# ZcsrenlongZ/Deblur4DGS

Measured on AMD Instinct MI355X. Metric: Gaussians/s fwd+bwd, 288x512, N_exposure=8, higher is better.
Workload: dtype f32; 1 GPU; cfg2: 300000 Gaussians (300000 dynamic), 6 motion bases, 512x288, N_exposure=8, 3+depth channels, fwd+bwd to all leaves; gaussians=300000, exposure_subsamples=8, parallelism=1 GPU, lazy_sort=off (auto), pre_roll_steps=30

## Files before the change

deblur4dgs_amd/csrc/binning.hip:

```cpp
#include "common.h"

namespace {

struct EmitArgs {
  D4gsDims d;
  const float *depths;
  const int32_t *tile_rects;
  const int32_t *tiles_touched;
  const int32_t *isect_offsets;
  int32_t *isect_offsets_out;
  const int32_t *chunk_base;
  int nchunks;
  int32_t *tile_cursor;
  const int32_t *tile_offsets;
  uint64_t *keys;
  int32_t *gid_of_emit;
  int tw, th;
  const int64_t *n_dev;
  int64_t cap, max_hint;
  int use_lds;
  LazyWs lazy;
  const uint64_t *tile_masks;
};

template <int EMIT_PER_THREAD, int LZ>
__global__ void __launch_bounds__(D4GS_CHUNK_THREADS) k_emit(const EmitArgs a) {
  extern __shared__ int bins[];
  if (lists_overflowed(a.n_dev, a.cap, a.max_hint)) return;
  constexpr bool LAZY = LZ != 0;
  const int tiles = a.tw * a.th, tid = threadIdx.x;
  const int s = blockIdx.x % a.d.S, chunk = blockIdx.x / a.d.S;
  const int tbase = s * tiles, n_tiles_all = a.d.S * tiles;
  const bool lds = a.use_lds;
  __shared__ int fbox[4];
  if (lds) {
    for (int z = tid; z < tiles; z += D4GS_CHUNK_THREADS) bins[z] = 0;
    if (LZ == 2 && tid == 0) fbox[0] = fbox[1] = 1 << 30, fbox[2] = fbox[3] = -1;
    __syncthreads();
  }
// ... 98 lines not shown
      __syncthreads();
      int base = 0, tot = 0;
#pragma unroll
      for (int w = 0; w < D4GS_CHUNK_THREADS / 64; w++) {
        const int x = wsum[w];
        base += w < wave ? x : 0;
        tot += x;
      }
      ebase[q] = (uint32_t)(carry + base + inc - cnt[q]);
      carry += tot;
      __syncthreads();
      const int g = (chunk * EMIT_PER_THREAD + q) * D4GS_CHUNK_THREADS + tid;
      if (g < a.d.N) a.isect_offsets_out[(int64_t)s * a.d.N + g] = (int32_t)ebase[q];
    }
  }
#pragma unroll
  for (int q = 0; q < EMIT_PER_THREAD; q++) {
    if (cnt[q] == 0) continue;
    const int g = (chunk * EMIT_PER_THREAD + q) * D4GS_CHUNK_THREADS + tid;
    const int64_t i = (int64_t)s * a.d.N + g;
    const int x0 = rx[q] & 0xffff, x1 = rx[q] >> 16, y0 = ry[q] & 0xffff, y1 = ry[q] >> 16;
    const uint64_t hi = (uint64_t)__float_as_uint(dep[q]) << 32;
    uint32_t e = (LZ != 2 && a.nchunks) ? ebase[q] : (uint32_t)a.isect_offsets[i];
    auto put = [&](int t) {
      if (LAZY && !taken(bkq[q], t)) return;
      const int slot = (LAZY || lds) ? atomicAdd(&bins[t], 1)
                                     : a.tile_offsets[tbase + t] + atomicAdd(a.tile_cursor + n_tiles_all + tbase + t, 1);
      a.keys[slot] = hi | e;
      a.gid_of_emit[e] = g;
    };
    if (msk[q]) {
      for (uint64_t m = msk[q]; m; m &= m - 1, e++) {
        const int b = __ffsll((long long)m) - 1;
        put((y0 + (b >> 3)) * a.tw + x0 + (b & 7));
      }
      continue;
    }
    for (int ty = y0; ty < y1; ty++)
      for (int tx = x0; tx < x1; tx++, e++) put(ty * a.tw + tx);
  }
}

__device__ __forceinline__ void bitonic_step(uint64_t *key, int P, int n, int k, int j) {
  for (int t = threadIdx.x; t < (P >> 1); t += blockDim.x) {
    const int blk = t / j, off = t - blk * j;
    const int i = blk * 2 * j + off;
    const int l = (j == (k >> 1)) ? (blk * 2 * j + (2 * j - 1 - off)) : (i + j);
    if (l < n) {
      const uint64_t x = key[i], y = key[l];
      if (x > y) key[i] = y, key[l] = x;
    }
  }
// ... 88 lines not shown
    reg_plain<NV, 1>(v);
    chunk_plain<32, NV>(v, lane);
  }
  if constexpr (NV >= 8) {
    reg_flip<NV, 8>(v);
    reg_plain<NV, 2>(v);
    chunk_plain<32, NV>(v, lane);
  }
}
constexpr int CNV = 8, CHUNK = 64 * CNV;

struct SortArgs {
  const int32_t *tile_offsets;
  uint64_t *keys;
  const int32_t *gid_of_emit;
  int32_t *sorted_gid;
  int32_t *sorted_emit;
  int lo, cap;
  const int64_t *n_dev;
  int64_t n_cap, max_hint;
  int n_lists;
  const int32_t *lazy_near, *lazy_flag;
  int pass;
};
__device__ __forceinline__ bool lazy_range(const SortArgs &a, int t, int &base, int &n) {
  if (a.pass == 1) n = min(n, a.lazy_near[t]);
  else if (a.pass == 2) {
    const int nn = a.lazy_near[t];
    if (nn >= n || a.lazy_flag[t] != 1) return false;
    base += nn, n -= nn;
  }
  return true;
}

__device__ __forceinline__ void put_sorted(const SortArgs &a, int at, uint64_t key) {
  const uint32_t e = (uint32_t)key;
  a.sorted_emit[at] = (int32_t)e;
  a.sorted_gid[at] = a.gid_of_emit[e];
}

template <int NV>
__device__ __forceinline__ void wave_sort_list(const SortArgs &a, int base, int n, int lane) {
  uint64_t v[NV];
  const uint64_t *gk = a.keys + base;
#pragma unroll
  for (int u = 0; u < NV; u++) v[u] = (u * 64 + lane < n) ? gk[u * 64 + lane] : ~0ull;
  chunk_sort<NV>(v, lane);
#pragma unroll
  for (int u = 0; u < NV; u++)
    if (u * 64 + lane < n) put_sorted(a, base + u * 64 + lane, v[u]);
}
__device__ __forceinline__ void wave_sort_list(const SortArgs &a, int base, int n, int lane) {
  if (n <= 64) wave_sort_list<1>(a, base, n, lane);
  else if (n <= 128) wave_sort_list<2>(a, base, n, lane);
  else if (n <= 256) wave_sort_list<4>(a, base, n, lane);
  else wave_sort_list<8>(a, base, n, lane);
}
template <int NV>
__device__ __forceinline__ void sort_list_lds(const SortArgs &a, uint64_t *key, int base, int n) {
// ... 76 lines not shown
    if (threadIdx.x < 64) wave_sort_list(a, base, n, threadIdx.x);
    return;
  }
  if (a.cap >= 0) {
    sort_list_lds(a, skeys, base, n);
  } else {
    uint64_t *gk = a.keys + base;
    bitonic_sort(gk, n);
    for (int p = threadIdx.x; p < n; p += blockDim.x) put_sorted(a, base + p, gk[p]);
  }
}


int launch_sorts(const D4gsDims *dims, const FrontPlan &fp, const D4gsProjOut *proj, const D4gsIsect *isect, int pass, hipStream_t stream) {
  const int n_tiles = fp.n_tiles;
  LazyWs lw{};
  if (pass) lw = d4gs_lazy_carve(proj->lazy_ws, dims->S, fp.tiles);
  (void)hipFuncSetAttribute((const void *)k_tile_sort, hipFuncAttributeMaxDynamicSharedMemorySize, 16384 * 8);
  const int64_t longest = isect->max_tile_count > 0 ? isect->max_tile_count : isect->n_isect;
  const bool merge_short = pass == 0 && longest > CHUNK && isect->n_isect >= (int64_t)768 * n_tiles;
  static const bool no_long = getenv("D4GS_SORT_NO_MERGE_LONG") != nullptr;
  const bool merge_long = !merge_short && !no_long && longest > CHUNK && pass == 0 && isect->n_isect < (int64_t)640 * n_tiles;
  SortArgs s{proj->tile_offsets, isect->keys, isect->gid_of_emit, isect->sorted_gid, isect->sorted_emit,
             0, CHUNK, proj->n_isect, isect->n_isect, isect->max_tile_count, n_tiles, lw.near, lw.flag, pass};
  if (!merge_short) {
    if (merge_long) D4GS_LAUNCH("k_tile_sort_w", k_tile_sort_w<true>, dim3((n_tiles + 3) / 4), dim3(256), 4 * CHUNK * 8, stream, s);
    else D4GS_LAUNCH("k_tile_sort_w", k_tile_sort_w<false>, dim3((n_tiles + 3) / 4), dim3(256), 0, stream, s);
  }
  const int classes[6][3] = {{merge_short ? 0 : CHUNK, 2048, 256}, {2048, 4096, 512}, {4096, 8192, 1024}, {8192, 16384, 1024}, {16384, -1, 1024}};
  for (int c = merge_long ? 1 : 0; c < 5; c++) {
    if (longest <= classes[c][0]) break;
    s.lo = classes[c][0], s.cap = classes[c][1];
    const size_t lds = classes[c][1] > 0 ? (size_t)classes[c][1] * 8 : 0;
    D4GS_LAUNCH("k_tile_sort", k_tile_sort, dim3(n_tiles), dim3(classes[c][2]), lds, stream, s);
  }
  return d4gs_check_launch("k_tile_sort");
}

EmitArgs emit_args(const D4gsDims *dims, const FrontPlan &fp, const D4gsProjOut *proj, const D4gsIsect *isect) {
  EmitArgs e;
  e.d = *dims;
  e.depths = proj->depths;
  e.tile_rects = proj->tile_rects;
  e.tiles_touched = proj->tiles_touched;
  e.isect_offsets = proj->isect_offsets;
  e.isect_offsets_out = proj->isect_offsets, e.chunk_base = proj->scan_ws, e.nchunks = fp.fused_chunks;
  e.tile_cursor = proj->tile_counts;
  e.tile_masks = (dims->flags & D4GS_EXACT_TILES) ? proj->tile_masks : nullptr;
  e.tile_offsets = proj->tile_offsets;
  e.keys = isect->keys;
  e.gid_of_emit = isect->gid_of_emit;
  e.tw = fp.tw, e.th = fp.th;
  e.n_dev = proj->n_isect, e.cap = isect->n_isect, e.max_hint = isect->max_tile_count;
  e.use_lds = fp.hist_in_lds;
  e.lazy = LazyWs{};
  return e;
}

int launch_emit(const EmitArgs &e, const FrontPlan &fp, int lz, hipStream_t stream) {
  const size_t ebytes = fp.hist_in_lds ? sizeof(int) * (size_t)fp.tiles * (lz ? 2 : 1) : 0;
  d4gs_with_pt(fp.pt, [&](auto pt) {
    constexpr int PT = decltype(pt)::value;
    d4gs_launch_chunks("k_emit", lz == 0 ? k_emit<PT, 0> : lz == 1 ? k_emit<PT, 1> : k_emit<PT, 2>, fp, ebytes, stream, e);
  });
  return d4gs_check_launch("k_emit");
}

}

int d4gs_bin_sort_impl(const D4gsDims *dims, const D4gsProjOut *proj, const D4gsIsect *isect, hipStream_t stream) {
  if (isect->n_isect <= 0) return D4GS_OK;
  if (isect->n_isect >= (int64_t)0x7fffffff) {
    d4gs_set_error("n_isect=%lld exceeds int32 indexing", (long long)isect->n_isect);
    return D4GS_ECAPACITY;
// ... 21 lines not shown
```

deblur4dgs_amd/csrc/capi.hip:

```cpp
#include <stdarg.h>
#include <stdio.h>
#include <string.h>

#include <stdint.h>

#include "common.h"

static thread_local char g_err[512] = "";

#include <mutex>
#include <string>
#include <vector>
namespace {
struct ProfRec {
  const char *name;
  hipEvent_t a, b;
};
int g_prof_on = 0;
std::vector<ProfRec> g_prof;
std::mutex g_prof_mu;
}

ProfScope::ProfScope(const char *name, hipStream_t s) : slot(-1), stream(s) {
  if (!g_prof_on) return;
// ... 46 lines not shown
  const bool flag = (d->flags & D4GS_ANTIALIASED) != 0;
  if (flag && !compensations) {
    d4gs_set_error("%s: D4GS_ANTIALIASED needs D4gsProjOut.compensations", who);
    return D4GS_EINVAL;
  }
  if (!flag && compensations) {
    d4gs_set_error("%s: D4gsProjOut.compensations given without D4GS_ANTIALIASED in dims->flags", who);
    return D4GS_EINVAL;
  }
  return D4GS_OK;
}

static int check_dims(const D4gsDims *d) {
  if (!d) {
    d4gs_set_error("dims is NULL");
    return D4GS_EINVAL;
  }
  if (d->D == 0 && d->depth_mode == D4GS_DEPTH_NONE) {
    d4gs_set_error("bad dims: D == 0 needs depth_mode D4GS_DEPTH_D or D4GS_DEPTH_ED (the depth-only render modes)");
    return D4GS_EINVAL;
  }
  if (d->N < 0 || d->S <= 0 || d->width <= 0 || d->height <= 0 || d->D < 0) {
    d4gs_set_error("bad dims N=%d S=%d W=%d H=%d D=%d", d->N, d->S, d->width, d->height, d->D);
    return D4GS_EINVAL;
  }
  if (d->G < 0 || d->G > d->N || (d->G > 0 && (d->K <= 0 || d->K > D4GS_MAX_K || d->T <= 0))) {
    d4gs_set_error("bad motion dims G=%d K=%d (max %d) T=%d", d->G, d->K, D4GS_MAX_K, d->T);
    return D4GS_EINVAL;
  }
  return D4GS_OK;
}

extern "C" {

int d4gs_version(void) { return D4GS_VERSION; }

__global__ void k_copy_counts(const int64_t *__restrict__ n_isect, int64_t *__restrict__ host_pinned) {
  if (threadIdx.x < 4) __hip_atomic_store(host_pinned + threadIdx.x, n_isect[threadIdx.x], __ATOMIC_RELAXED, __HIP_MEMORY_SCOPE_SYSTEM);
}
}
int d4gs_copy_counts_impl(const int64_t *n_isect, int64_t *host_pinned, hipStream_t stream) {
  if (!n_isect || !host_pinned) {
    d4gs_set_error("d4gs_copy_counts: NULL argument");
    return D4GS_EINVAL;
  }
  hipPointerAttribute_t at{};
// ... 474 lines not shown
```

deblur4dgs_amd/csrc/frame.hip:

```cpp
#include "common.h"

namespace {

struct Carve {
  char *base;
  size_t off;
  template <typename T>
  T *take(size_t n) {
    off = (off + 255) & ~(size_t)255;
    T *p = base ? reinterpret_cast<T *>(base + off) : nullptr;
    off += n * sizeof(T);
    return p;
  }
};

struct FrameBufs {
  D4gsProjOut proj;
  D4gsIsect isect;
  D4gsRaster raster;
  float *v_renders, *v_alphas, *isect_grad, *v_conics, *v_depths, *v_opac_act, *v_ctab, *partials;
  uint8_t *isect_live;
  int8_t *blend_win;
  size_t bytes;
  size_t fwd_bytes;
// ... 43 lines not shown
    d4gs_set_error("%s: S=%d sub-samples with a blended frame, the one-call frame takes at most %d (its winner map holds one signed byte "
                   "per pixel and channel); use the staged entry points", who, d->S, D4GS_FRAME_BLEND_MAX_S);
    return D4GS_EINVAL;
  }
  if (!in || !io || !ws || !io->renders || !io->alphas || !io->means2d || !io->radii || !io->n_isect ||
      (io->blended && !io->acc) || !in->means || !in->quats || !in->scales || !in->opacities || !in->colors || !in->viewmat ||
      !in->Kmat || (d->G > 0 && (!in->motion_coefs || !in->rots || !in->transls || !in->times)) || d->N == 0) {
    d4gs_set_error("%s: NULL required buffer", who);
    return D4GS_EINVAL;
  }
  if (((uintptr_t)ws & 255) != 0) {
    d4gs_set_error("%s: the workspace must be 256-byte aligned", who);
    return D4GS_EINVAL;
  }
  const FrameBufs need = carve(d, cap, nullptr);
  if (ws_bytes < (forward_only ? need.fwd_bytes : need.bytes)) {
    d4gs_set_error("%s: workspace of %zu bytes, need %zu (%s)", who, ws_bytes, forward_only ? need.fwd_bytes : need.bytes,
                   forward_only ? "d4gs_frame_workspace_bytes_fwd; d4gs_backward needs d4gs_frame_workspace_bytes" : "d4gs_frame_workspace_bytes");
    return D4GS_ECAPACITY;
  }
  return D4GS_OK;
}

void bind_io(FrameBufs &b, const D4gsFrameIO *io, int64_t cap, int64_t max_hint) {
  b.proj.means2d = io->means2d, b.proj.radii = io->radii, b.proj.n_isect = io->n_isect;
  b.isect.n_isect = cap > 0 ? cap : 1, b.isect.max_tile_count = max_hint, b.isect.near_target = io->near_target;
  b.raster.background = io->background, b.raster.render_colors = io->renders, b.raster.render_alphas = io->alphas;
}

}

extern "C" {

size_t d4gs_frame_workspace_bytes(const D4gsDims *dims, int64_t isect_capacity) {
  D4gsSizes z;
  if (d4gs_query_sizes(dims, &z)) return 0;
  if (dims->D == 0) {
    frame_refuses_depth_only("d4gs_frame_workspace_bytes");
    return 0;
  }
  return carve(dims, isect_capacity, nullptr).bytes;
}

size_t d4gs_frame_workspace_bytes_fwd(const D4gsDims *dims, int64_t isect_capacity) {
  D4gsSizes z;
  if (d4gs_query_sizes(dims, &z)) return 0;
  if (dims->D == 0) {
    frame_refuses_depth_only("d4gs_frame_workspace_bytes_fwd");
    return 0;
  }
  return carve(dims, isect_capacity, nullptr).fwd_bytes;
}

int d4gs_forward(const D4gsDims *dims, const D4gsProjIn *in, const D4gsFrameIO *io, void *ws, size_t ws_bytes,
                 int64_t isect_capacity, int64_t max_tile_hint, void *stream_) {
  int rc = check_frame("d4gs_forward", dims, in, io, ws, ws_bytes, isect_capacity, true);
  if (rc) return rc;
  hipStream_t stream = (hipStream_t)stream_;
  if (io->counts_pinned) {
    hipPointerAttribute_t at{};
    if (hipPointerGetAttributes(&at, io->counts_pinned) != hipSuccess || at.type != hipMemoryTypeHost) {
      (void)hipGetLastError();
      d4gs_set_error("d4gs_forward: io->counts_pinned is not pinned host memory");
      return D4GS_EINVAL;
    }
  }
  FrameBufs b = carve(dims, isect_capacity, ws);
  bind_io(b, io, isect_capacity, max_tile_hint);
  if ((rc = d4gs_project_fwd_impl(dims, in, &b.proj, stream))) return rc;
  if (isect_capacity < 0)
    return io->counts_pinned ? d4gs_copy_counts_impl(io->n_isect, io->counts_pinned, stream) : D4GS_OK;
  if ((rc = d4gs_bin_sort_impl(dims, &b.proj, &b.isect, stream))) return rc;
  if ((rc = d4gs_raster_fwd_impl(dims, &b.proj, &b.isect, &b.raster, stream))) return rc;
  if (io->blended) {
    rc = d4gs_blend_fwd_impl(dims->S, (int64_t)dims->width * dims->height, d4gs_nch(dims), io->policy, io->renders, io->alphas, io->blended,
                             io->acc, b.blend_win, stream,
                             io->n_isect, io->counts_pinned);
  } else if (io->counts_pinned) {
    rc = d4gs_copy_counts_impl(io->n_isect, io->counts_pinned, stream);
  }
  return rc;
}

int d4gs_backward(const D4gsDims *dims, const D4gsProjIn *in, const D4gsFrameIO *io, const D4gsFrameGrads *g,
                  const D4gsLeafGrads *leaf, void *ws, size_t ws_bytes, int64_t isect_capacity, int64_t max_tile_hint,
                  void *stream_) {
  int rc = check_frame("d4gs_backward", dims, in, io, ws, ws_bytes, isect_capacity);
  if (rc) return rc;
  if (!g || !leaf || !g->v_means2d || !leaf->v_means || !leaf->v_quats || !leaf->v_scales || !leaf->v_opacities ||
      !leaf->v_colors || (dims->G > 0 && (!leaf->v_motion_coefs || !leaf->v_rots || !leaf->v_transls)) ||
      (io->blended ? (!g->v_blended && !g->v_acc && !g->v_renders && !g->v_alphas) : !g->v_renders)) {
    d4gs_set_error("d4gs_backward: NULL gradient buffer (a blended frame takes any of v_blended, v_acc, v_renders, v_alphas; an "
                   "unblended one v_renders [+ v_alphas])");
    return D4GS_EINVAL;
  }
  if ((rc = d4gs_check_absgrad("d4gs_backward", dims, g->v_means2d_abs, g->stats_absgrad))) return rc;
  hipStream_t stream = (hipStream_t)stream_;
  FrameBufs b = carve(dims, isect_capacity, ws);
  bind_io(b, io, isect_capacity, max_tile_hint);
  const float *v_renders = g->v_renders, *v_alphas = g->v_alphas;
  const int nch = d4gs_nch(dims);
  const bool fuse_blend = io->blended && !g->v_renders && !g->v_alphas && dims->D <= 5;
  BlendAdj ba{};
  if (fuse_blend) {
    ba.v_blended = g->v_blended, ba.v_acc = g->v_acc, ba.win = b.blend_win;
    for (int c = 0; c < nch; c++)
      if (io->policy && io->policy[c] != 0) ba.non_mean |= (uint64_t)1 << c;
    v_renders = nullptr, v_alphas = nullptr;
  } else if (io->blended) {
    if ((rc = d4gs_blend_bwd_add_impl(dims->S, (int64_t)dims->width * dims->height, nch, io->policy, io->renders, io->blended,
                                      g->v_blended, g->v_acc, b.v_renders, b.v_alphas, g->v_renders, g->v_alphas, stream,
                                      b.blend_win)))
      return rc;
    v_renders = b.v_renders, v_alphas = b.v_alphas;
  }
  D4gsRasterGrads rg{};
  rg.v_render_colors = v_renders, rg.v_render_alphas = v_alphas, rg.isect_grad = b.isect_grad, rg.isect_live = b.isect_live;
  rg.v_means2d = g->v_means2d, rg.v_conics = b.v_conics, rg.v_depths = b.v_depths, rg.v_opac_act = b.v_opac_act;
  rg.v_ctab = b.v_ctab;
  rg.stats_grad_norm_acc = g->stats_grad_norm_acc, rg.stats_vis_count = g->stats_vis_count;
  rg.stats_max_radii = g->stats_max_radii, rg.stats_batch_size = g->stats_batch_size;
  rg.stats_update_max_radii = g->stats_update_max_radii, rg.row_mode = g->row_mode;
// ... 13 lines not shown
```

deblur4dgs_amd/csrc/host.h:

```cpp
#pragma once
#include <hip/hip_runtime_api.h>
#include <stddef.h>
#include <stdint.h>

#include "../../include/d4gs.h"

void d4gs_set_error(const char *fmt, ...);
int d4gs_check_launch(const char *what);
int d4gs_check_absgrad(const char *who, const D4gsDims *d, const float *v_means2d_abs, int32_t stats_absgrad);
int d4gs_check_antialiased(const char *who, const D4gsDims *d, const float *compensations);
int d4gs_copy_counts_impl(const int64_t *n_isect, int64_t *host_pinned, hipStream_t stream);

int d4gs_project_fwd_impl(const D4gsDims *dims, const D4gsProjIn *in, const D4gsProjOut *out, hipStream_t stream);
int d4gs_project_bwd_impl(const D4gsDims *dims, const D4gsProjIn *in, const D4gsProjOut *proj, const float *v_means2d,
                          const float *v_conics, const float *v_depths, const float *v_opac_act, const float *v_ctab,
                          const D4gsLeafGrads *grads, hipStream_t stream);
int d4gs_poses_fwd_impl(const D4gsDims *dims, const D4gsProjIn *in, const D4gsPoses *out, hipStream_t stream);
int d4gs_poses_bwd_impl(const D4gsDims *dims, const D4gsProjIn *in, const D4gsPoses *v_out, const D4gsLeafGrads *grads,
                        hipStream_t stream);
size_t d4gs_poses_bwd_partials_bound(const D4gsDims *d);
int d4gs_bases_table_launch(const D4gsDims *dims, const D4gsProjIn *in, float *btab, hipStream_t stream);
inline int d4gs_tiles_across(int pixels) { return (pixels + D4GS_TILE - 1) / D4GS_TILE; }
inline int d4gs_nch(const D4gsDims *d) { return d->D + (d->depth_mode != D4GS_DEPTH_NONE ? 1 : 0); }

constexpr int D4GS_CHUNK_THREADS = 1024;
static_assert(D4GS_CHUNK_THREADS % 64 == 0 && D4GS_CHUNK_THREADS <= 1024, "whole waves, one workgroup");
struct FrontPlan {
  int tw, th, tiles;
  int n_tiles;
  bool hist_in_lds;
  bool count_apart;
  int pt, per_block, nchunks , blocks ;
  int fused_chunks;
};
FrontPlan d4gs_front_plan(const D4gsDims *d);

int d4gs_bin_sort_impl(const D4gsDims *dims, const D4gsProjOut *proj, const D4gsIsect *isect, hipStream_t stream);
bool d4gs_lazy_on(const D4gsDims *d, const D4gsProjOut *out, const FrontPlan &fp);
int d4gs_lazy_pivot_launch(const D4gsDims *d, const D4gsProjOut *out, const FrontPlan &fp, int64_t near_target, hipStream_t stream);
int d4gs_lazy_far_sort(const D4gsDims *dims, const D4gsProjOut *proj, const D4gsIsect *isect, hipStream_t stream);

struct BlendAdj {
  const float *v_blended;
  const float *v_acc;
  const int8_t *win;
  uint64_t non_mean;
};
int d4gs_raster_fwd_impl(const D4gsDims *dims, const D4gsProjOut *proj, const D4gsIsect *isect, const D4gsRaster *r,
                         hipStream_t stream);
int d4gs_raster_bwd_impl(const D4gsDims *dims, const D4gsProjOut *proj, const D4gsIsect *isect, const D4gsRaster *r,
                         const D4gsRasterGrads *g, const BlendAdj *blend, hipStream_t stream);
int64_t d4gs_seg_state_elems(const D4gsDims *d);
bool d4gs_seg_on(const D4gsDims *d, const D4gsIsect *isect, const D4gsRaster *r);

int d4gs_blend_fwd_impl(int32_t S, int64_t P, int32_t C, const int32_t *policy, const float *renders, const float *alphas,
                        float *out, float *acc, int8_t *win, hipStream_t stream, const int64_t *n_isect = nullptr,
                        int64_t *counts_pinned = nullptr);
// ... 44 lines not shown
```

deblur4dgs_amd/csrc/project_fwd.hip:

```cpp
#include <stdlib.h>

#include "common.h"

namespace {

struct FwdArgs {
  D4gsDims d;
  D4gsProjIn in;
  D4gsProjOut out;
  int tw, th;
  int count_apart;
  int use_table;
};

__device__ __forceinline__ void preblend_bases(const FwdArgs &a, float *Bs) {
#pragma clang fp contract(off)
  const int K = a.d.K, T = a.d.T;
  for (int idx = threadIdx.x; idx < a.d.S * K * 9; idx += blockDim.x) {
    int s = idx / (K * 9), r = idx - s * K * 9, k = r / 9, j = r - k * 9;
    const TimeSlot ts = d4gs_time_slot(a.in.times[s], T);
    const float w = ts.w;
    const int f = ts.f, c = ts.c;
    float vf, vc;
    if (j < 3) {
// ... 655 lines not shown
  static const bool force_in_kernel = getenv("D4GS_COUNT_IN_PROJECT") != nullptr;
  static const bool no_fused_scan = getenv("D4GS_NO_FUSED_SCAN") != nullptr;
  FrontPlan p;
  p.tw = d4gs_tiles_across(d->width), p.th = d4gs_tiles_across(d->height);
  p.tiles = p.tw * p.th, p.n_tiles = d->S * p.tiles;
  p.hist_in_lds = sizeof(int) * (size_t)p.tiles <= 64 * 1024;
  p.count_apart = p.hist_in_lds && d->N > 0 && !force_in_kernel;
  auto blocks_at = [&](int pt) { return (((int64_t)d->N + (int64_t)pt * D4GS_CHUNK_THREADS - 1) / ((int64_t)pt * D4GS_CHUNK_THREADS)) * d->S; };
  p.pt = 4;
  if (blocks_at(4) < 256) {
    p.pt = 1;
  } else if (!(d->flags & D4GS_LAZY_SORT)) {
    for (int pt = 2; pt <= 6; pt++)
      if (blocks_at(pt) <= 512) {
        p.pt = pt;
        break;
      }
  }
  p.per_block = D4GS_CHUNK_THREADS * p.pt;
  p.nchunks = (d->N + p.per_block - 1) / p.per_block;
  p.blocks = p.nchunks * d->S;
  const bool fits = (size_t)p.blocks + 1 <= d4gs_scan_ws_elems((int64_t)d->S * d->N);
  p.fused_chunks = p.count_apart && !no_fused_scan && fits ? p.nchunks : 0;
  return p;
}

bool d4gs_lazy_on(const D4gsDims *d, const D4gsProjOut *out, const FrontPlan &fp) {
  if (!(d->flags & D4GS_LAZY_SORT) || !out->lazy_ws) return false;
  return fp.count_apart && sizeof(int) * (size_t)fp.tiles * (1 + d4gs_lazy_buckets(fp.tiles)) <= 150 * 1024;
}
int d4gs_lazy_pivot_launch(const D4gsDims *d, const D4gsProjOut *out, const FrontPlan &fp, int64_t near_target, hipStream_t stream) {
  const int target = near_target > 0 ? (int)(near_target > (1 << 20) ? (1 << 20) : near_target) : 1024;
  D4GS_LAUNCH("k_lazy_pivot", k_lazy_pivot, dim3((fp.n_tiles + 255) / 256), dim3(256), 0, stream, d4gs_lazy_carve(out->lazy_ws, d->S, fp.tiles),
              fp.n_tiles, target);
  return d4gs_check_launch("k_lazy_pivot");
}

static size_t fwd_lds_bytes(const D4gsDims *dims) {
  if (dims->G <= 0) return 0;
  return sizeof(float) * (((size_t)dims->S * dims->K * 9 + 3) & ~(size_t)3) + sizeof(float) * (size_t)dims->K * D4GS_PROJ_BLOCK;
}

int d4gs_poses_fwd_impl(const D4gsDims *dims, const D4gsProjIn *in, const D4gsPoses *out, hipStream_t stream) {
  PosesArgs a;
  a.d = *dims;
  a.in = *in;
// ... 90 lines not shown
```

deblur4dgs_amd/csrc/raster_bwd.hip:

```cpp
#include <stdlib.h>

#include <type_traits>

#include "composite.h"

namespace {

struct RasterBwdArgs {
  int N, S, width, height, tw, th;
  int ed;
  const float *geom;
  const float *ctab;
  const float *background;
  const int32_t *tile_offsets;
  const int32_t *sorted_gid;
  const int32_t *sorted_emit;
  const float *out;
  const float *alphas;
  const int32_t *last_ids;
  const float *final_T;
  const float *v_out;
  const float *v_alphas;
  float *isect_grad;
  uint8_t *live;
  int sparse;
  const int64_t *n_dev;
  int64_t cap, max_hint;
  const float *seg_state;
  int fuse_blend;
  BlendAdj blend;
#ifdef D4GS_TRACE
  unsigned long long *trace;
#endif
};
#ifdef D4GS_TRACE
#define D4GS_TRACE_BEGIN const unsigned long long _t0 = wall_clock64();
#define D4GS_TRACE_END(n_)                                                                                     \
  if (a.trace && threadIdx.x == 0) {                                                                           \
    unsigned long long *tr = a.trace + (size_t)blockIdx.x * 4;                                                 \
// ... 119 lines not shown
      if (last >= end) {
        const float *sf = a.seg_state + (size_t)t * D4GS_SEG_MAX * (1 + NCH) * 256 + ((y - ty * D4GS_TILE) * D4GS_TILE + (x - tx * D4GS_TILE));
        const float *sb = sf + (size_t)(seg + 1) * (1 + NCH) * 256;
        T = sb[0];
#pragma unroll
        for (int c = 0; c < NCH; c++) bsum = __builtin_fmaf(vo[c], sf[(1 + c) * 256] - sb[(1 + c) * 256], bsum);
        last = end - 1;
      }
    }
  }
  int whi = last < start ? start - 1 : last;
  int wq = whi;
#pragma unroll
  for (int o = 1; o <= 16; o = o == 2 ? 8 : o << 1) wq = max(wq, __shfl_xor(wq, o));
  const int wq0 = __builtin_amdgcn_readlane(wq, 0), wq1 = __builtin_amdgcn_readlane(wq, 4), wq2 = __builtin_amdgcn_readlane(wq, 32),
            wq3 = __builtin_amdgcn_readlane(wq, 36);
#pragma unroll
  for (int o = 32; o > 0; o >>= 1) whi = max(whi, __shfl_xor(whi, o));
  whi = min(whi, end - 1);
  if (lane == 0) shi[wv] = whi;
  __syncthreads();
  const int hi = max(max(shi[0], shi[1]), max(shi[2], shi[3]));
  const size_t inst_base = (size_t)s * a.N;
  float *myslab = sgrad + wv * NB * RP;
  const int wvs = __builtin_amdgcn_readfirstlane(wv);
  float afrag[MC ? 16 : 1];
  float *myfac = sfac + (MC ? wv * 64 * FS : 0);
  int *myhit = shit + (MC ? wv * MH : 0);
  int nh = 0;
  if constexpr (MC > 0) {
    static_assert(256 * MC <= 4 * NB * RP, "exchange buffer");
#pragma unroll
    for (int c = 0; c < MC; c++) sgrad[tid * MC + c] = vo[c];
    __syncthreads();
#pragma unroll
    for (int kk = 0; kk < 16; kk++) afrag[kk] = sgrad[(wv * 64 + 4 * kk + (lane >> 4)) * MC + (lane & 15)];
  }
  auto flush = [&](int nhits) {
    if constexpr (MC > 0) {
      __builtin_amdgcn_wave_barrier();
      f32x4 acc0 = {0.f, 0.f, 0.f, 0.f}, acc1 = {0.f, 0.f, 0.f, 0.f};
      const float *bp = myfac + (lane >> 4) * FS + (lane & (MH - 1));
      float bv[16];
#pragma unroll
      for (int kk = 0; kk < 16; kk++) bv[kk] = bp[4 * kk * FS];
#pragma unroll
      for (int kk = 0; kk < 16; kk += 2) {
        acc0 = __builtin_amdgcn_mfma_f32_16x16x4f32(afrag[kk], bv[kk], acc0, 0, 0, 0);
        acc1 = __builtin_amdgcn_mfma_f32_16x16x4f32(afrag[kk + 1], bv[kk + 1], acc1, 0, 0, 0);
      }
      acc0 += acc1;
      const int n = lane & 15;
      if (n < nhits) {
        float *dst = myslab + myhit[n] * RP + CB + (lane >> 4) * 4;
        dst[0] = acc0[0], dst[1] = acc0[1], dst[2] = acc0[2], dst[3] = acc0[3];
      }
      __builtin_amdgcn_wave_barrier();
    }
  };
  if (!a.sparse)
    for (int idx = hi + 1 + tid; idx < end; idx += 256) {
      float *dst = a.isect_grad + (size_t)a.sorted_emit[idx] * RW;
#pragma unroll
      for (int r = 0; r < RW; r++) dst[r] = 0.f;
    }

  float vab = va - bsum;
  for (int bh = hi; bh >= start; bh -= NB) {
    __syncthreads();
    int emit = -1;
    if (tid < NB) {
      const int idx = bh - tid;
      if (idx >= start) {
        const int gid = a.sorted_gid[idx];
        emit = a.sorted_emit[idx];
        const float4 *gp = reinterpret_cast<const float4 *>(a.geom + (inst_base + gid) * D4GS_GEOM_STRIDE);
        const float4 q0 = gp[0], q1 = gp[1];
        sg0[tid] = q0;
        sg1[tid] = stage_conic(q1.x, q1.y, q1.z, __builtin_amdgcn_rcpf(q0.z));
        const float tau = D4GS_ALPHA_TAU(q0.z);
        D4GS_TIGHT_EXTENTS(ex, ey, tau, q1.x, q1.y, q1.z)
        if constexpr (W4)
          sbox[tid] = ex < 0.f ? d4gs_pack_box(1e30f, -1e30f, 1e30f, -1e30f)
                               : d4gs_pack_box(q0.x - ex - tx0f, q0.x + ex - tx0f, q0.y - ey - ty0f, q0.y + ey - ty0f);
        else
          sbox[tid] = ex < 0.f ? make_float4(1e30f, -1e30f, 1e30f, -1e30f)
                               : make_float4(q0.x - ex, q0.x + ex, q0.y - ey, q0.y + ey);
        const float4 *cp = reinterpret_cast<const float4 *>(a.ctab + (size_t)gid * DP);
#pragma unroll
        for (int v = 0; v < DV; v++) {
          float4 c4 = cp[v];
          if constexpr (DEPTH && (D & 3) != 0) {
            if (v == D / 4) (&c4.x)[D & 3] = q0.w;
          }
          scol[tid * DV + v] = c4;
        }
      }
    }
    for (int z = tid; z < NB * RP; z += 256) reinterpret_cast<float4 *>(sgrad)[z] = make_float4(0.f, 0.f, 0.f, 0.f);
    __syncthreads();
// ... 419 lines not shown
  a.v_opac_act[g] = vo;
#pragma unroll
  for (int c = 0; c < DP; c++) a.v_ctab[(size_t)g * DP + c] = c < D ? vc[c < D ? c : 0] : 0.f;
}

static bool choose_sparse(int row_mode, int64_t n_isect, int64_t n_inst, bool lazy) {
  if (lazy) return true;
  if (row_mode == D4GS_ROWS_DENSE) return false;
  if (row_mode == D4GS_ROWS_SPARSE) return true;
  return n_isect >= 6 * (n_inst > 0 ? n_inst : 1);
}

template <int D, bool DEPTH, bool ABS, bool AA>
int launch_bwd(RasterBwdArgs &a, GatherArgs &ga, const GatherAA &gaa, int64_t n_isect, int row_mode, bool lazy, hipStream_t stream) {
  const int n_tiles = a.S * a.tw * a.th;
  const int blocks = ((n_tiles + 7) / 8) * 8;
  bool launched = false;
  a.sparse = ga.sparse = choose_sparse(row_mode, n_isect, (int64_t)a.S * a.N, lazy) ? 1 : 0;
#ifdef D4GS_VARIANTS
  static const bool wave_per_tile = getenv("D4GS_BWD_WAVE_PER_TILE") != nullptr;
  static const bool use_mfma = getenv("D4GS_BWD_MFMA") != nullptr;
  if constexpr (D > 0) {
    if (!ABS && (wave_per_tile || use_mfma)) {
      constexpr int R = 6 + D + (DEPTH ? 1 : 0);
      a.sparse = ga.sparse = 0;
      if (wave_per_tile) {
        hipError_t e = hipMemsetAsync(a.isect_grad, 0, sizeof(float) * (size_t)R * (size_t)(n_isect > 0 ? n_isect : 1), stream);
        if (e != hipSuccess) {
          d4gs_set_error("hipMemsetAsync(isect_grad): %s", hipGetErrorString(e));
          return D4GS_ELAUNCH;
        }
      }
      if (n_isect > 0) {
        if (wave_per_tile) D4GS_LAUNCH("k_raster_bwd", (k_raster_bwd<D, DEPTH>), dim3(blocks), dim3(64), 0, stream, a);
        else D4GS_LAUNCH("k_raster_bwd_m", (k_raster_bwd_m<D, DEPTH>), dim3(blocks), dim3(256), 0, stream, a);
      }
      launched = true;
    }
  }
#endif
  if (!launched) {
    if (a.sparse) {
      hipError_t e = hipMemsetAsync(a.live, 0, (((size_t)(n_isect > 0 ? n_isect : 1)) + 3) & ~(size_t)3, stream);
      if (e != hipSuccess) {
        d4gs_set_error("hipMemsetAsync(isect_live): %s", hipGetErrorString(e));
        return D4GS_ELAUNCH;
// ... 22 lines not shown
    else D4GS_GATHER(true, 1);
  } else {
    if (slots == 4) D4GS_GATHER(false, 4);
    else if (slots == 2) D4GS_GATHER(false, 2);
    else D4GS_GATHER(false, 1);
  }
#undef D4GS_GATHER
  return d4gs_check_launch("k_gather");
}

}

int d4gs_raster_bwd_impl(const D4gsDims *dims, const D4gsProjOut *proj, const D4gsIsect *isect, const D4gsRaster *r,
                         const D4gsRasterGrads *g, const BlendAdj *blend, hipStream_t stream) {
  RasterBwdArgs a;
  a.fuse_blend = blend != nullptr;
  a.blend = blend ? *blend : BlendAdj{};
  a.N = dims->N, a.S = dims->S, a.width = dims->width, a.height = dims->height;
  const FrontPlan fp = d4gs_front_plan(dims);
  a.tw = fp.tw, a.th = fp.th;
  a.ed = dims->depth_mode == D4GS_DEPTH_ED;
  a.geom = proj->geom, a.ctab = proj->ctab, a.background = r->background;
  a.tile_offsets = proj->tile_offsets, a.sorted_gid = isect->sorted_gid, a.sorted_emit = isect->sorted_emit;
  a.out = r->render_colors, a.alphas = r->render_alphas, a.last_ids = r->last_ids, a.final_T = r->final_T;
  a.v_out = g->v_render_colors, a.v_alphas = g->v_render_alphas, a.isect_grad = g->isect_grad, a.live = g->isect_live;
  a.n_dev = proj->n_isect, a.cap = isect->n_isect, a.max_hint = isect->max_tile_count;
  a.seg_state = d4gs_seg_on(dims, isect, r) ? r->seg_state : nullptr;
#ifdef D4GS_TRACE
  a.trace = getenv("D4GS_TRACE_PTR") ? (unsigned long long *)strtoull(getenv("D4GS_TRACE_PTR"), nullptr, 0) : nullptr;
#endif
  GatherArgs ga;
  ga.n_dev = proj->n_isect, ga.cap = isect->n_isect, ga.max_hint = isect->max_tile_count;
  ga.rows = isect->n_isect > 0 ? isect->n_isect : 1;
  ga.live = g->isect_live;
  ga.N = dims->N, ga.S = dims->S, ga.D = dims->D, ga.DP = (dims->D + 3) & ~3;
  ga.depth = dims->depth_mode != D4GS_DEPTH_NONE;
  ga.tiles_touched = proj->tiles_touched, ga.isect_offsets = proj->isect_offsets, ga.isect_grad = g->isect_grad;
  ga.v_means2d = g->v_means2d, ga.v_conics = g->v_conics, ga.v_depths = g->v_depths, ga.v_opac_act = g->v_opac_act;
  ga.v_ctab = g->v_ctab;
  ga.radii = proj->radii, ga.stats_acc = g->stats_grad_norm_acc, ga.stats_vis = g->stats_vis_count;
  ga.stats_mr = g->stats_max_radii, ga.update_mr = g->stats_update_max_radii;
  ga.sx = (float)dims->width / 2.0f * (float)g->stats_batch_size * (float)dims->S;
  ga.sy = (float)dims->height / 2.0f * (float)g->stats_batch_size * (float)dims->S;
  const bool absg = (dims->flags & D4GS_ABSGRAD) != 0;
  ga.v_means2d_abs = absg ? g->v_means2d_abs : nullptr, ga.stats_abs = absg && g->stats_absgrad;
  ga.max_wh = (float)(dims->width > dims->height ? dims->width : dims->height);
// ... 117 lines not shown
```

deblur4dgs_amd/csrc/raster_fwd.hip:

```cpp
#include <stdlib.h>

#include "composite.h"

namespace {

struct RasterFwdArgs {
  int N, S, width, height, tw, th;
  int ed;
  const float *geom;
  const float *ctab;
  const float *background;
  const int32_t *tile_offsets;
  const int32_t *sorted_gid;
  float *out;
  float *alphas;
  int32_t *last_ids;
  float *final_T;
  int64_t *n_dev;
  int64_t cap, max_hint;
  float *seg_state;
  const int32_t *lazy_near;
  int32_t *lazy_flag;
  int lazy_pass;
  int block_filter;
#ifdef D4GS_TRACE
  unsigned long long *trace;
#endif
};
#ifdef D4GS_TRACE
#define D4GS_TCLK(v_) const unsigned long long v_ = wall_clock64();
#define D4GS_TADD(acc_, a_, b_) acc_ += (b_) - (a_);
// ... 96 lines not shown
  } else if (a.lazy_pass == 2 && !a.lazy_flag[t]) return;
  const size_t inst_base = (size_t)s * a.N;
  const int seglen = SEG ? d4gs_seg_len(end_full - start) : 0;
  float *seg_px = SEG ? a.seg_state + (size_t)t * D4GS_SEG_MAX * (1 + NCH) * 256 + ((y - ty * D4GS_TILE) * D4GS_TILE + (x - tx * D4GS_TILE)) : nullptr;
  auto seg_store = [&](int k) {
    if (inside) {
      float *p = seg_px + (size_t)k * (1 + NCH) * 256;
      p[0] = T;
#pragma unroll
      for (int c = 0; c < NCH; c++) p[(1 + c) * 256] = chan(c);
    }
  };
  for (int b = start; b < end; b += FBE) {
    if (__syncthreads_and(done)) break;
    D4GS_TCLK(_ta)
    const int idx = b + tid - (NULL0 ? 1 : 0);
    if (NULL0 && tid == 0) {
      sg0[0] = make_float4(0.f, 0.f, 0.f, 0.f);
      sg1[0] = make_float4(0.f, 0.f, 0.f, 0.f);
      sbox[0] = BoxT<PB>::pack(1e30f, -1e30f, 1e30f, -1e30f);
#pragma unroll
      for (int v = 0; v < DV; v++) scol[v] = make_float4(0.f, 0.f, 0.f, 0.f);
    } else if (tid < FB && idx < end) {
      const int gid = a.sorted_gid[idx];
      const float4 *gp = reinterpret_cast<const float4 *>(a.geom + (inst_base + gid) * D4GS_GEOM_STRIDE);
      const float4 q0 = gp[0], q1 = gp[1];
      sg0[tid] = q0;
      const float tau = d4gs_alpha_tau(q0.z);
      sg1[tid] = stage_conic(q1.x, q1.y, q1.z, tau * 1.4426950408889634f);
      D4GS_TIGHT_EXTENTS(ex, ey, tau, q1.x, q1.y, q1.z)
      sbox[tid] = ex < 0.f ? BoxT<PB>::pack(1e30f, -1e30f, 1e30f, -1e30f) : BoxT<PB>::pack(q0.x - ex - tx0f, q0.x + ex - tx0f, q0.y - ey - ty0f, q0.y + ey - ty0f);
      const float4 *cp = reinterpret_cast<const float4 *>(a.ctab + (size_t)gid * DP);
#pragma unroll
      for (int v = 0; v < DV; v++) scol[tid * DV + v] = cp[v];
    }
    __syncthreads();
    D4GS_TCLK(_tb)
    D4GS_TADD(_ts, _ta, _tb)
    const bool wave_live = __builtin_amdgcn_ballot_w64(done) != ~0ull;
    const int nb = wave_live ? min(FBE, end - b) + (NULL0 ? 1 : 0) : 0;
    int c0 = 0, c1 = 0, c2 = 0, c3 = 0;
    if constexpr (NARROW) {
      if (lane * 16 < 4 * FB) reinterpret_cast<uint4 *>(wlist)[lane] = make_uint4(0u, 0u, 0u, 0u);
      __builtin_amdgcn_wave_barrier();
    }
#pragma unroll
    for (int k = 0; k < FB / 64; k++) {
// ... 194 lines not shown
  raster_fwd_r_body<D, DEPTH>(a);
}
template <int D, bool DEPTH>
__global__ void __launch_bounds__(256) __attribute__((amdgpu_waves_per_eu(D == 16 ? 6 : 1, D == 16 ? 6 : 10))) k_raster_fwd_r(const RasterFwdArgs a) {
  raster_fwd_r_body<D, DEPTH>(a);
}
template <int D, bool DEPTH>
__global__ void __launch_bounds__(256) __attribute__((amdgpu_waves_per_eu(8, 8))) k_raster_fwd_rs8(const RasterFwdArgs a) {
  raster_fwd_r_body<D, DEPTH, true>(a);
}
template <int D, bool DEPTH>
__global__ void __launch_bounds__(256) __attribute__((amdgpu_waves_per_eu(D == 16 ? 6 : 1, D == 16 ? 6 : 10))) k_raster_fwd_rs(const RasterFwdArgs a) {
  raster_fwd_r_body<D, DEPTH, true>(a);
}

template <int D, bool DEPTH>
int launch_fwd(const RasterFwdArgs &a, hipStream_t stream) {
  const int n_tiles = a.S * a.tw * a.th;
  const int blocks = ((n_tiles + 7) / 8) * 8;
#ifdef D4GS_VARIANTS
  static const bool wave_per_tile = getenv("D4GS_FWD_WAVE_PER_TILE") != nullptr;
  static const bool quads = getenv("D4GS_FWD_QUADS") != nullptr;
  if constexpr (D > 0) {
    if (wave_per_tile) {
      D4GS_LAUNCH("k_raster_fwd", (k_raster_fwd<D, DEPTH>), dim3(blocks), dim3(64), 0, stream, a);
      return d4gs_check_launch("k_raster_fwd");
    }
    if (quads) {
      D4GS_LAUNCH("k_raster_fwd_q", (k_raster_fwd_q<D, DEPTH>), dim3(blocks), dim3(256), 0, stream, a);
      return d4gs_check_launch("k_raster_fwd_q");
    }
  }
#endif
  if (a.seg_state) {
    if constexpr (D <= 4) D4GS_LAUNCH("k_raster_fwd_r", (k_raster_fwd_rs8<D, DEPTH>), dim3(blocks), dim3(256), 0, stream, a);
    else D4GS_LAUNCH("k_raster_fwd_r", (k_raster_fwd_rs<D, DEPTH>), dim3(blocks), dim3(256), 0, stream, a);
    return d4gs_check_launch("k_raster_fwd_r");
  }
  if constexpr (D <= 4) D4GS_LAUNCH("k_raster_fwd_r", (k_raster_fwd_r8<D, DEPTH>), dim3(blocks), dim3(256), 0, stream, a);
  else D4GS_LAUNCH("k_raster_fwd_r", (k_raster_fwd_r<D, DEPTH>), dim3(blocks), dim3(256), 0, stream, a);
  return d4gs_check_launch("k_raster_fwd_r");
}

}

int64_t d4gs_seg_state_elems(const D4gsDims *d) {
// ... 1 lines not shown
  if (n_tiles > (d->D <= 4 ? D4GS_SEG_TILES_MAX_NARROW : D4GS_SEG_TILES_MAX)) return 0;
  return n_tiles * D4GS_SEG_MAX * (1 + d4gs_nch(d)) * 256;
}
bool d4gs_seg_on(const D4gsDims *d, const D4gsIsect *isect, const D4gsRaster *r) {
  const char *env = getenv("D4GS_SEG");
  if (!r->seg_state || d4gs_seg_state_elems(d) == 0 || (env && env[0] == '0')) return false;
#ifdef D4GS_VARIANTS
  if (getenv("D4GS_FWD_WAVE_PER_TILE") || getenv("D4GS_FWD_QUADS") || getenv("D4GS_BWD_WAVE_PER_TILE") || getenv("D4GS_BWD_MFMA"))
    return false;
#endif
  if (env && env[0] == '1') return true;
  return isect->max_tile_count > D4GS_SEG_UNIT;
}

int d4gs_raster_fwd_impl(const D4gsDims *dims, const D4gsProjOut *proj, const D4gsIsect *isect, const D4gsRaster *r,
                         hipStream_t stream) {
  RasterFwdArgs a;
  a.N = dims->N, a.S = dims->S, a.width = dims->width, a.height = dims->height;
  const FrontPlan fp = d4gs_front_plan(dims);
  a.tw = fp.tw, a.th = fp.th;
  a.ed = dims->depth_mode == D4GS_DEPTH_ED;
  a.geom = proj->geom, a.ctab = proj->ctab, a.background = r->background;
  a.tile_offsets = proj->tile_offsets, a.sorted_gid = isect->sorted_gid;
  a.n_dev = proj->n_isect, a.cap = isect->n_isect, a.max_hint = isect->max_tile_count;
  a.out = r->render_colors, a.alphas = r->render_alphas, a.last_ids = r->last_ids, a.final_T = r->final_T;
  a.seg_state = d4gs_seg_on(dims, isect, r) ? r->seg_state : nullptr;
  a.lazy_near = nullptr, a.lazy_flag = nullptr, a.lazy_pass = 0;
  const char *bf = getenv("D4GS_BLOCK_FILTER");
  a.block_filter = !(bf && bf[0] == '0');
  const bool lazy = d4gs_lazy_on(dims, proj, fp) && isect->n_isect > 0;
  if (lazy) {
    const LazyWs lw = d4gs_lazy_carve(proj->lazy_ws, dims->S, fp.tiles);
    a.lazy_near = lw.near, a.lazy_flag = lw.flag, a.lazy_pass = 1;
  }
#ifdef D4GS_TRACE
  a.trace = getenv("D4GS_TRACE_FWD_PTR") ? (unsigned long long *)strtoull(getenv("D4GS_TRACE_FWD_PTR"), nullptr, 0) : nullptr;
#endif
  const bool dep = dims->depth_mode != D4GS_DEPTH_NONE;
  auto launch = [&](const RasterFwdArgs &aa) -> int {
#define D4GS_CASE(DD)                                                   \
  case DD:                                                              \
    return dep ? launch_fwd<DD, true>(aa, stream) : launch_fwd<DD, false>(aa, stream);
    switch (dims->D) {
      case 0:
        if (dep) return launch_fwd<0, true>(aa, stream);
        d4gs_set_error("D = 0 needs a depth mode (the depth-only composite)");
// ... 39 lines not shown
```

Baseline: 253.7 million Gaussians/s.

## Pack gaussian id and per-gaussian ordinal into sort key low word

In the one-call frame path, the low 32 bits of each intersection key hold the gaussian id shifted left plus a per-gaussian tile ordinal, instead of a global emit index. This drops the gid_of_emit scatter in emit, the gather through gid_of_emit in the sort, and the sorted_emit writes. Backward rebuilds the emit index from isect_offsets plus the ordinal when it needs it. It only applies when N and the tile count fit together in 32 bits and lazy sort is off, and the reference raster variants are rejected when it is active.

```diff
diff --git a/deblur4dgs_amd/csrc/binning.hip b/deblur4dgs_amd/csrc/binning.hip
--- a/deblur4dgs_amd/csrc/binning.hip
+++ b/deblur4dgs_amd/csrc/binning.hip
@@ -15,6 +15,7 @@
   const int32_t *tile_offsets;
   uint64_t *keys;
   int32_t *gid_of_emit;
+  int ordbits;
   int tw, th;
   const int64_t *n_dev;
   int64_t cap, max_hint;
@@ -159,12 +160,14 @@
     const int x0 = rx[q] & 0xffff, x1 = rx[q] >> 16, y0 = ry[q] & 0xffff, y1 = ry[q] >> 16;
     const uint64_t hi = (uint64_t)__float_as_uint(dep[q]) << 32;
     uint32_t e = (LZ != 2 && a.nchunks) ? ebase[q] : (uint32_t)a.isect_offsets[i];
+    const bool packed = !LAZY && a.ordbits != 0;
+    if (packed) e = (uint32_t)g << a.ordbits;
     auto put = [&](int t) {
       if (LAZY && !taken(bkq[q], t)) return;
       const int slot = (LAZY || lds) ? atomicAdd(&bins[t], 1)
                                      : a.tile_offsets[tbase + t] + atomicAdd(a.tile_cursor + n_tiles_all + tbase + t, 1);
       a.keys[slot] = hi | e;
-      a.gid_of_emit[e] = g;
+      if (!packed) a.gid_of_emit[e] = g;
     };
     if (msk[q]) {
       for (uint64_t m = msk[q]; m; m &= m - 1, e++) {
@@ -299,6 +302,7 @@
   int n_lists;
   const int32_t *lazy_near, *lazy_flag;
   int pass;
+  int packed;
 };
 __device__ __forceinline__ bool lazy_range(const SortArgs &a, int t, int &base, int &n) {
   if (a.pass == 1) n = min(n, a.lazy_near[t]);
@@ -312,6 +316,10 @@
 
 __device__ __forceinline__ void put_sorted(const SortArgs &a, int at, uint64_t key) {
   const uint32_t e = (uint32_t)key;
+  if (a.packed) {
+    a.sorted_gid[at] = (int32_t)e;
+    return;
+  }
   a.sorted_emit[at] = (int32_t)e;
   a.sorted_gid[at] = a.gid_of_emit[e];
 }
@@ -434,7 +442,7 @@
   static const bool no_long = getenv("D4GS_SORT_NO_MERGE_LONG") != nullptr;
   const bool merge_long = !merge_short && !no_long && longest > CHUNK && pass == 0 && isect->n_isect < (int64_t)640 * n_tiles;
   SortArgs s{proj->tile_offsets, isect->keys, isect->gid_of_emit, isect->sorted_gid, isect->sorted_emit,
-             0, CHUNK, proj->n_isect, isect->n_isect, isect->max_tile_count, n_tiles, lw.near, lw.flag, pass};
+             0, CHUNK, proj->n_isect, isect->n_isect, isect->max_tile_count, n_tiles, lw.near, lw.flag, pass, fp.packed_ids ? 1 : 0};
   if (!merge_short) {
     if (merge_long) D4GS_LAUNCH("k_tile_sort_w", k_tile_sort_w<true>, dim3((n_tiles + 3) / 4), dim3(256), 4 * CHUNK * 8, stream, s);
     else D4GS_LAUNCH("k_tile_sort_w", k_tile_sort_w<false>, dim3((n_tiles + 3) / 4), dim3(256), 0, stream, s);
@@ -462,6 +470,7 @@
   e.tile_offsets = proj->tile_offsets;
   e.keys = isect->keys;
   e.gid_of_emit = isect->gid_of_emit;
+  e.ordbits = fp.packed_ids ? fp.ordbits : 0;
   e.tw = fp.tw, e.th = fp.th;
   e.n_dev = proj->n_isect, e.cap = isect->n_isect, e.max_hint = isect->max_tile_count;
   e.use_lds = fp.hist_in_lds;
diff --git a/deblur4dgs_amd/csrc/capi.hip b/deblur4dgs_amd/csrc/capi.hip
--- a/deblur4dgs_amd/csrc/capi.hip
+++ b/deblur4dgs_amd/csrc/capi.hip
@@ -92,6 +92,10 @@
   }
   if (d->N < 0 || d->S <= 0 || d->width <= 0 || d->height <= 0 || d->D < 0) {
     d4gs_set_error("bad dims N=%d S=%d W=%d H=%d D=%d", d->N, d->S, d->width, d->height, d->D);
+    return D4GS_EINVAL;
+  }
+  if (d->flags & D4GS_FRAME_PACKED_IDS) {
+    d4gs_set_error("bad dims: flags bit 0x%x is not a public flag", (unsigned)D4GS_FRAME_PACKED_IDS);
     return D4GS_EINVAL;
   }
   if (d->G < 0 || d->G > d->N || (d->G > 0 && (d->K <= 0 || d->K > D4GS_MAX_K || d->T <= 0))) {
diff --git a/deblur4dgs_amd/csrc/frame.hip b/deblur4dgs_amd/csrc/frame.hip
--- a/deblur4dgs_amd/csrc/frame.hip
+++ b/deblur4dgs_amd/csrc/frame.hip
@@ -89,6 +89,12 @@
   return D4GS_OK;
 }
 
+D4gsDims frame_dims(const D4gsDims *dims) {
+  D4gsDims d = *dims;
+  d.flags |= D4GS_FRAME_PACKED_IDS;
+  return d;
+}
+
 void bind_io(FrameBufs &b, const D4gsFrameIO *io, int64_t cap, int64_t max_hint) {
   b.proj.means2d = io->means2d, b.proj.radii = io->radii, b.proj.n_isect = io->n_isect;
   b.isect.n_isect = cap > 0 ? cap : 1, b.isect.max_tile_count = max_hint, b.isect.near_target = io->near_target;
@@ -134,6 +140,8 @@
   }
   FrameBufs b = carve(dims, isect_capacity, ws);
   bind_io(b, io, isect_capacity, max_tile_hint);
+  const D4gsDims fd = frame_dims(dims);
+  dims = &fd;
   if ((rc = d4gs_project_fwd_impl(dims, in, &b.proj, stream))) return rc;
   if (isect_capacity < 0)
     return io->counts_pinned ? d4gs_copy_counts_impl(io->n_isect, io->counts_pinned, stream) : D4GS_OK;
@@ -165,6 +173,8 @@
   hipStream_t stream = (hipStream_t)stream_;
   FrameBufs b = carve(dims, isect_capacity, ws);
   bind_io(b, io, isect_capacity, max_tile_hint);
+  const D4gsDims fd = frame_dims(dims);
+  dims = &fd;
   const float *v_renders = g->v_renders, *v_alphas = g->v_alphas;
   const int nch = d4gs_nch(dims);
   const bool fuse_blend = io->blended && !g->v_renders && !g->v_alphas && dims->D <= 5;
diff --git a/deblur4dgs_amd/csrc/host.h b/deblur4dgs_amd/csrc/host.h
--- a/deblur4dgs_amd/csrc/host.h
+++ b/deblur4dgs_amd/csrc/host.h
@@ -32,7 +32,10 @@
   bool count_apart;
   int pt, per_block, nchunks , blocks ;
   int fused_chunks;
+  int idbits, ordbits;
+  bool packed_ids;
 };
+constexpr int32_t D4GS_FRAME_PACKED_IDS = 1 << 30;
 FrontPlan d4gs_front_plan(const D4gsDims *d);
 
 int d4gs_bin_sort_impl(const D4gsDims *dims, const D4gsProjOut *proj, const D4gsIsect *isect, hipStream_t stream);
diff --git a/deblur4dgs_amd/csrc/project_fwd.hip b/deblur4dgs_amd/csrc/project_fwd.hip
--- a/deblur4dgs_amd/csrc/project_fwd.hip
+++ b/deblur4dgs_amd/csrc/project_fwd.hip
@@ -701,6 +701,15 @@
   p.blocks = p.nchunks * d->S;
   const bool fits = (size_t)p.blocks + 1 <= d4gs_scan_ws_elems((int64_t)d->S * d->N);
   p.fused_chunks = p.count_apart && !no_fused_scan && fits ? p.nchunks : 0;
+  static const bool no_packed_ids = [] {
+    const char *e = getenv("D4GS_PACKED_IDS");
+    return e && e[0] == '0';
+  }();
+  p.idbits = 1;
+  while (p.idbits < 31 && ((int64_t)1 << p.idbits) < (int64_t)d->N) p.idbits++;
+  p.ordbits = 32 - p.idbits;
+  p.packed_ids = (d->flags & D4GS_FRAME_PACKED_IDS) && !no_packed_ids && !(d->flags & D4GS_LAZY_SORT) &&
+                 (int64_t)p.tiles <= ((int64_t)1 << p.ordbits);
   return p;
 }
 
diff --git a/deblur4dgs_amd/csrc/raster_bwd.hip b/deblur4dgs_amd/csrc/raster_bwd.hip
--- a/deblur4dgs_amd/csrc/raster_bwd.hip
+++ b/deblur4dgs_amd/csrc/raster_bwd.hip
@@ -9,12 +9,14 @@
 struct RasterBwdArgs {
   int N, S, width, height, tw, th;
   int ed;
+  int ordbits;
   const float *geom;
   const float *ctab;
   const float *background;
   const int32_t *tile_offsets;
   const int32_t *sorted_gid;
   const int32_t *sorted_emit;
+  const int32_t *isect_offsets;
   const float *out;
   const float *alphas;
   const int32_t *last_ids;
@@ -180,6 +182,9 @@
   __syncthreads();
   const int hi = max(max(shi[0], shi[1]), max(shi[2], shi[3]));
   const size_t inst_base = (size_t)s * a.N;
+  auto packed_emit = [&](uint32_t word) -> int {
+    return a.isect_offsets[inst_base + (word >> a.ordbits)] + (int)(word & ((1u << a.ordbits) - 1u));
+  };
   float *myslab = sgrad + wv * NB * RP;
   const int wvs = __builtin_amdgcn_readfirstlane(wv);
   float afrag[MC ? 16 : 1];
@@ -218,7 +223,7 @@
   };
   if (!a.sparse)
     for (int idx = hi + 1 + tid; idx < end; idx += 256) {
-      float *dst = a.isect_grad + (size_t)a.sorted_emit[idx] * RW;
+      float *dst = a.isect_grad + (size_t)(a.ordbits ? packed_emit((uint32_t)a.sorted_gid[idx]) : a.sorted_emit[idx]) * RW;
 #pragma unroll
       for (int r = 0; r < RW; r++) dst[r] = 0.f;
     }
@@ -230,10 +235,13 @@
     if (tid < NB) {
       const int idx = bh - tid;
       if (idx >= start) {
-        const int gid = a.sorted_gid[idx];
-        emit = a.sorted_emit[idx];
+        const uint32_t word = (uint32_t)a.sorted_gid[idx];
+        const int gid = (int)(word >> a.ordbits);
         const float4 *gp = reinterpret_cast<const float4 *>(a.geom + (inst_base + gid) * D4GS_GEOM_STRIDE);
+        const int32_t *rp = a.ordbits ? a.isect_offsets + (inst_base + gid) : a.sorted_emit + idx;
+        const int row0 = *rp;
         const float4 q0 = gp[0], q1 = gp[1];
+        emit = row0 + (int)(word & ((1u << a.ordbits) - 1u));
         sg0[tid] = q0;
         sg1[tid] = stage_conic(q1.x, q1.y, q1.z, __builtin_amdgcn_rcpf(q0.z));
         const float tau = D4GS_ALPHA_TAU(q0.z);
@@ -699,6 +707,10 @@
   static const bool use_mfma = getenv("D4GS_BWD_MFMA") != nullptr;
   if constexpr (D > 0) {
     if (!ABS && (wave_per_tile || use_mfma)) {
+      if (a.ordbits) {
+        d4gs_set_error("the reference variants of the composite backward do not take the one-call frame's packed-id lists (set D4GS_PACKED_IDS=0)");
+        return D4GS_EINVAL;
+      }
       constexpr int R = 6 + D + (DEPTH ? 1 : 0);
       a.sparse = ga.sparse = 0;
       if (wave_per_tile) {
@@ -767,6 +779,7 @@
   a.ed = dims->depth_mode == D4GS_DEPTH_ED;
   a.geom = proj->geom, a.ctab = proj->ctab, a.background = r->background;
   a.tile_offsets = proj->tile_offsets, a.sorted_gid = isect->sorted_gid, a.sorted_emit = isect->sorted_emit;
+  a.isect_offsets = proj->isect_offsets, a.ordbits = fp.packed_ids ? fp.ordbits : 0;
   a.out = r->render_colors, a.alphas = r->render_alphas, a.last_ids = r->last_ids, a.final_T = r->final_T;
   a.v_out = g->v_render_colors, a.v_alphas = g->v_render_alphas, a.isect_grad = g->isect_grad, a.live = g->isect_live;
   a.n_dev = proj->n_isect, a.cap = isect->n_isect, a.max_hint = isect->max_tile_count;
diff --git a/deblur4dgs_amd/csrc/raster_fwd.hip b/deblur4dgs_amd/csrc/raster_fwd.hip
--- a/deblur4dgs_amd/csrc/raster_fwd.hip
+++ b/deblur4dgs_amd/csrc/raster_fwd.hip
@@ -7,6 +7,7 @@
 struct RasterFwdArgs {
   int N, S, width, height, tw, th;
   int ed;
+  int ordbits;
   const float *geom;
   const float *ctab;
   const float *background;
@@ -149,7 +150,7 @@
 #pragma unroll
       for (int v = 0; v < DV; v++) scol[v] = make_float4(0.f, 0.f, 0.f, 0.f);
     } else if (tid < FB && idx < end) {
-      const int gid = a.sorted_gid[idx];
+      const int gid = (int)((uint32_t)a.sorted_gid[idx] >> a.ordbits);
       const float4 *gp = reinterpret_cast<const float4 *>(a.geom + (inst_base + gid) * D4GS_GEOM_STRIDE);
       const float4 q0 = gp[0], q1 = gp[1];
       sg0[tid] = q0;
@@ -390,6 +391,10 @@
   static const bool wave_per_tile = getenv("D4GS_FWD_WAVE_PER_TILE") != nullptr;
   static const bool quads = getenv("D4GS_FWD_QUADS") != nullptr;
   if constexpr (D > 0) {
+    if ((wave_per_tile || quads) && a.ordbits) {
+      d4gs_set_error("the reference variants of the forward composite do not take the one-call frame's packed-id lists (set D4GS_PACKED_IDS=0)");
+      return D4GS_EINVAL;
+    }
     if (wave_per_tile) {
       D4GS_LAUNCH("k_raster_fwd", (k_raster_fwd<D, DEPTH>), dim3(blocks), dim3(64), 0, stream, a);
       return d4gs_check_launch("k_raster_fwd");
@@ -437,6 +442,7 @@
   a.ed = dims->depth_mode == D4GS_DEPTH_ED;
   a.geom = proj->geom, a.ctab = proj->ctab, a.background = r->background;
   a.tile_offsets = proj->tile_offsets, a.sorted_gid = isect->sorted_gid;
+  a.ordbits = fp.packed_ids ? fp.ordbits : 0;
   a.n_dev = proj->n_isect, a.cap = isect->n_isect, a.max_hint = isect->max_tile_count;
   a.out = r->render_colors, a.alphas = r->render_alphas, a.last_ids = r->last_ids, a.final_T = r->final_T;
   a.seg_state = d4gs_seg_on(dims, isect, r) ? r->seg_state : nullptr;
```

Result: no change. 255.5 million Gaussians/s, median of 6 (+0.7%).
